# allegro/allRank

Measured on NVIDIA H100. Metric: slates/sec, higher is better.
Workload: dtype tf32

## Files before the change

allrank_b200/csrc/ffn_chain.cu:

```cuda
#include <algorithm>
#include <cstdio>
#include <cuda.h>
#include <cuda_runtime.h>

#include "common.h"
#include "gemm_tf32.h"
#include "sm90_ptx.cuh"

namespace arb {

namespace {

constexpr int CH_ROWS = 128;
constexpr int CH_UNITS = 64;
constexpr int UNIT_BYTES = 64 * 128;
constexpr int X_SLAB_BYTES = CH_ROWS * 128;
constexpr int H_SLAB_BYTES = 64 * 128;
constexpr int CH_THREADS = 384;
constexpr int SMEM_LIMIT = 227 * 1024;

template <int D>
struct ChainLayout {
  static constexpr int KB1 = D / 32;
  static constexpr int NBU = (D + 63) / 64;
  static constexpr int X_BYTES = KB1 * X_SLAB_BYTES;
  static constexpr int H_BYTES = 2 * 2 * H_SLAB_BYTES;
  static constexpr int TAIL_BYTES = 1024;
  static constexpr int NU_FIT = (SMEM_LIMIT - 1024 - TAIL_BYTES - X_BYTES - H_BYTES) / UNIT_BYTES;
  static constexpr int NU = NU_FIT < 16 ? NU_FIT : 16;
  static constexpr int RING_OFF = X_BYTES + H_BYTES;
  static constexpr int TAIL_OFF = RING_OFF + NU * UNIT_BYTES;
  static constexpr int total() { return TAIL_OFF + TAIL_BYTES + 1024; }
  static_assert(D % 32 == 0 && D >= 32 && D <= 256, "d: a multiple of 32 up to 256");
  static_assert(NU >= 2 * NBU, "the ring holds at least one k-block of the second product");
  static_assert(total() <= SMEM_LIMIT, "shared memory budget");
};

struct ChainParams {
  int M;
  int F;
  int rnd;
  int store_h;
  const float* b1;
  const float* b2;
  const float* aux;
  float* y;
  uint32_t* bits;
  float* colsum;
  const int* rows_dev;
};

__device__ __forceinline__ void load_a(uint32_t (&a)[4][4], const uint8_t* slab, int r0, int rnd) {
  const int lane = threadIdx.x & 31, j = lane >> 3;
#pragma unroll
  for (int ks = 0; ks < 4; ++ks) {
    ptx::ldmatrix_x4(a[ks], slab + ptx::sw128(r0 + 8 * (j & 1) + (lane & 7), 32 * ks + 16 * (j >> 1)));
    if (rnd) {
#pragma unroll
      for (int e = 0; e < 4; ++e) a[ks][e] = ptx::cvt_tf32(__uint_as_float(a[ks][e]));
    }
  }
}

template <int D, int U = 0>
__device__ __forceinline__ void second_mma(float (&acc)[D / 8][4], const uint32_t (&a)[4],
                                           const uint64_t (&desc)[(D + 63) / 64], int ks) {
  constexpr int WN = D % 64 == 0 ? 64 : 32;
  if constexpr (U < D / WN) {
    if constexpr (WN == 64) ptx::wgmma_m64n64k8_tf32<8 * U>(acc, a, desc[U] + 2 * ks);
    else ptx::wgmma_m64n32k8_tf32<4 * U>(acc, a, desc[U / 2] + (U & 1) * (32 * 128 / 16) + 2 * ks);
    second_mma<D, U + 1>(acc, a, desc, ks);
  }
}

template <int D, bool BWD>
__global__ void __launch_bounds__(CH_THREADS, 1) ffn_chain_kernel(const __grid_constant__ CUtensorMap tmX,
                                                                 const __grid_constant__ CUtensorMap tmA,
                                                                 const __grid_constant__ CUtensorMap tmB,
                                                                 const __grid_constant__ CUtensorMap tmH,
                                                                 const ChainParams p) {
  using L = ChainLayout<D>;
  constexpr int NU = L::NU, KB1 = L::KB1, NBU = L::NBU, NTY = D / 8;
  extern __shared__ uint8_t smem_dyn[];
  uint8_t* smem = reinterpret_cast<uint8_t*>((reinterpret_cast<uintptr_t>(smem_dyn) + 1023) & ~uintptr_t(1023));
  uint8_t* xs = smem;
  uint8_t* ring = smem + L::RING_OFF;
  uint64_t* full = reinterpret_cast<uint64_t*>(smem + L::TAIL_OFF);
  uint64_t* empty = full + NU;
  uint64_t* xfull = empty + NU;
  uint64_t* xfree = xfull + 8;
  uint64_t* csfull = xfree + 1;
  uint64_t* csempty = csfull + 2;
  float* csx = reinterpret_cast<float*>(smem + L::TAIL_OFF + 512);

  const int warp = threadIdx.x >> 5, lane = threadIdx.x & 31;
  if (threadIdx.x == 0) {
    ptx::prefetch_tmap(&tmX);
    ptx::prefetch_tmap(&tmA);
    ptx::prefetch_tmap(&tmB);
    if (p.store_h) ptx::prefetch_tmap(&tmH);
    for (int s = 0; s < NU; ++s) { ptx::mbar_init(&full[s], 1); ptx::mbar_init(&empty[s], 8); }
    for (int kb = 0; kb < KB1; ++kb) ptx::mbar_init(&xfull[kb], 1);
    ptx::mbar_init(xfree, 8);
    for (int b = 0; b < 2; ++b) { ptx::mbar_init(&csfull[b], 128); ptx::mbar_init(&csempty[b], 128); }
    ptx::fence_barrier_init();
  }
  arb_pdl_wait();
  __syncthreads();
  int n_tiles = (p.M + CH_ROWS - 1) / CH_ROWS;
  if (p.rows_dev) n_tiles = min(n_tiles, (__ldg(p.rows_dev) + CH_ROWS - 1) / CH_ROWS);
  const int n_chunks = p.F / CH_UNITS;

  if (warp >= 8) {
    asm volatile("setmaxnreg.dec.sync.aligned.u32 40;" ::: "memory");
    if (warp == 8 && lane == 0) {
      uint32_t it = 0;
      auto unit = [&](const CUtensorMap* tm, int c0, int c1) {
        const int s = it % NU;
        const uint32_t round = it / NU;
        if (round > 0) ptx::mbar_wait(&empty[s], (round - 1) & 1);
        ptx::mbar_expect_tx(&full[s], UNIT_BYTES);
        ptx::tma_load_4d(ring + s * UNIT_BYTES, tm, &full[s], c0, c1, 0, 0);
        ++it;
      };
      int local = 0;
      for (int t = blockIdx.x; t < n_tiles; t += gridDim.x, ++local) {
        const int m0 = t * CH_ROWS;
        if (local > 0) ptx::mbar_wait(xfree, (local - 1) & 1);
        for (int kb = 0; kb < KB1; ++kb) {
          ptx::mbar_expect_tx(&xfull[kb], X_SLAB_BYTES);
          ptx::tma_load_4d(xs + kb * X_SLAB_BYTES, &tmX, &xfull[kb], 32 * kb, m0, 0, 0);
        }
        if (!BWD) {
          const long long bytes = (long long)(min(p.M, m0 + CH_ROWS) - m0) * D * 4;
          asm volatile("cp.async.bulk.prefetch.L2.global [%0], %1;"
                       ::"l"(p.aux + (long long)m0 * D), "r"(uint32_t(bytes)) : "memory");
        }
        for (int j = 0; j < n_chunks; ++j) {
          for (int kb = 0; kb < KB1; ++kb) unit(&tmA, 32 * kb, CH_UNITS * j);
          for (int kb2 = 0; kb2 < 2; ++kb2)
            for (int u = 0; u < NBU; ++u) unit(&tmB, CH_UNITS * j + 32 * kb2, 64 * u);
        }
      }
    }
  } else {
    asm volatile("setmaxnreg.inc.sync.aligned.u32 232;" ::: "memory");
    const int g = warp >> 2, w = warp & 3, gq = lane >> 2, t4 = lane & 3, gt = threadIdx.x & 127;
    uint8_t* hs = smem + L::X_BYTES + g * 2 * H_SLAB_BYTES;
    const int fw = p.F >> 5;
    uint32_t it = 0, cj = 0;
    int local = 0;
    for (int t = blockIdx.x; t < n_tiles; t += gridDim.x, ++local) {
      const int m0 = t * CH_ROWS;
      const int row0 = m0 + 64 * g + 16 * w + gq;
      float accY[NTY][4];
#pragma unroll
      for (int n = 0; n < NTY; ++n) accY[n][0] = accY[n][1] = accY[n][2] = accY[n][3] = 0.f;
#pragma unroll 1
      for (int j = 0; j < n_chunks; ++j, ++cj) {
        uint32_t mw[2][2] = {{0u, 0u}, {0u, 0u}};
        if constexpr (BWD) {
#pragma unroll
          for (int h = 0; h < 2; ++h)
            if (row0 + 8 * h < p.M) {
              mw[h][0] = __ldg(p.bits + (long long)(row0 + 8 * h) * fw + 2 * j);
              mw[h][1] = __ldg(p.bits + (long long)(row0 + 8 * h) * fw + 2 * j + 1);
            }
        }
        float accH[8][4];
#pragma unroll
        for (int n = 0; n < 8; ++n) accH[n][0] = accH[n][1] = accH[n][2] = accH[n][3] = 0.f;
#pragma unroll 1
        for (int kb = 0; kb < KB1; ++kb, ++it) {
          const int s = it % NU;
          ptx::mbar_wait(&full[s], (it / NU) & 1);
          if (j == 0) ptx::mbar_wait(&xfull[kb], local & 1);
          uint32_t a[4][4];
          load_a(a, xs + kb * X_SLAB_BYTES, 64 * g + 16 * w, p.rnd);
          const uint64_t desc = ptx::wgmma_desc_sw128(ring + s * UNIT_BYTES);
          ptx::wgmma_fence_acc(accH);
          ptx::wgmma_fence();
#pragma unroll
          for (int ks = 0; ks < 4; ++ks) ptx::wgmma_m64n64k8_tf32<0>(accH, a[ks], desc + 2 * ks);
          ptx::wgmma_commit();
          ptx::wgmma_wait0();
          ptx::wgmma_fence_acc(accH);
          __syncwarp();
          if (lane == 0) ptx::mbar_arrive(&empty[s]);
        }
        if (j == n_chunks - 1) {
          __syncwarp();
          if (lane == 0) ptx::mbar_arrive(xfree);
        }
        if (p.store_h && lane == 0) ptx::tma_store_wait_read<0>();
        if (BWD && p.colsum) ptx::named_bar_sync(1 + g, 128);
        __syncwarp();
        uint32_t wb[2][2] = {{0u, 0u}, {0u, 0u}};
#pragma unroll
        for (int n = 0; n < 8; ++n) {
          const int c = 8 * n + 2 * t4, bp = 8 * (n & 3) + 2 * t4;
          float2 bb = make_float2(0.f, 0.f);
          if constexpr (!BWD) bb = __ldg(reinterpret_cast<const float2*>(p.b1 + CH_UNITS * j + c));
#pragma unroll
          for (int h = 0; h < 2; ++h) {
            float o0 = accH[n][2 * h], o1 = accH[n][2 * h + 1];
            if constexpr (BWD) {
              o0 = (mw[h][n >> 2] >> bp) & 1u ? o0 : 0.f;
              o1 = (mw[h][n >> 2] >> (bp + 1)) & 1u ? o1 : 0.f;
            } else {
              o0 += bb.x; o1 += bb.y;
              o0 = fmaxf(o0, 0.0f); o1 = fmaxf(o1, 0.0f);
              wb[h][n >> 2] |= (o0 > 0.f ? 1u : 0u) << bp | (o1 > 0.f ? 1u : 0u) << (bp + 1);
            }
            *reinterpret_cast<float2*>(hs + (n >> 2) * H_SLAB_BYTES + ptx::sw128(16 * w + gq + 8 * h, 4 * (c & 31))) =
                make_float2(o0, o1);
          }
        }
        if (!BWD && p.bits) {
#pragma unroll
          for (int h = 0; h < 2; ++h)
#pragma unroll
            for (int s = 0; s < 2; ++s) {
              wb[h][s] |= __shfl_xor_sync(0xffffffffu, wb[h][s], 1);
              wb[h][s] |= __shfl_xor_sync(0xffffffffu, wb[h][s], 2);
            }
          const int h = t4 >> 1, s = t4 & 1;
          const uint32_t word = t4 == 0 ? wb[0][0] : t4 == 1 ? wb[0][1] : t4 == 2 ? wb[1][0] : wb[1][1];
          if (row0 + 8 * h < p.M) p.bits[(long long)(row0 + 8 * h) * fw + 2 * j + s] = word;
        }
        if (p.store_h) ptx::fence_proxy_async_smem();
        __syncwarp();
        if (p.store_h && lane == 0) {
#pragma unroll
          for (int s = 0; s < 2; ++s)
            ptx::tma_store_4d(&tmH, hs + s * H_SLAB_BYTES + 16 * w * 128, CH_UNITS * j + 32 * s, m0 + 64 * g + 16 * w, 0, 0);
          ptx::tma_store_commit();
        }
        if constexpr (BWD) {
          if (p.colsum) {
            ptx::named_bar_sync(1 + g, 128);
            const int cc = gt >> 1, seg = gt & 1, c5 = cc & 31;
            const uint8_t* slab = hs + (cc >> 5) * H_SLAB_BYTES;
            float ts = 0.f;
#pragma unroll 8
            for (int r = 32 * seg; r < 32 * seg + 32; ++r)
              ts += *reinterpret_cast<const float*>(slab + r * 128 + ((((c5 >> 2) ^ (r & 7)) << 4) | ((c5 & 3) << 2)));
            ts += __shfl_xor_sync(0xffffffffu, ts, 1);
            const int b = cj & 1;
            const uint32_t use = cj >> 1;
            if (g == 1) {
              if (use > 0) ptx::mbar_wait(&csempty[b], (use - 1) & 1);
              if (seg == 0) csx[b * 64 + cc] = ts;
              ptx::mbar_arrive(&csfull[b]);
            } else {
              ptx::mbar_wait(&csfull[b], use & 1);
              const float other = csx[b * 64 + cc];
              ptx::mbar_arrive(&csempty[b]);
              if (seg == 0) p.colsum[(long long)t * p.F + CH_UNITS * j + cc] = ts + other;
            }
          }
        }
#pragma unroll 1
        for (int kb2 = 0; kb2 < 2; ++kb2, it += NBU) {
          uint32_t a[4][4];
          load_a(a, hs + kb2 * H_SLAB_BYTES, 16 * w, p.rnd);
          uint64_t desc[NBU];
#pragma unroll
          for (int u = 0; u < NBU; ++u) {
            const uint32_t iu = it + u;
            ptx::mbar_wait(&full[iu % NU], (iu / NU) & 1);
            desc[u] = ptx::wgmma_desc_sw128(ring + (iu % NU) * UNIT_BYTES);
          }
          ptx::wgmma_fence_acc(accY);
          ptx::wgmma_fence();
#pragma unroll
          for (int ks = 0; ks < 4; ++ks) second_mma<D>(accY, a[ks], desc, ks);
          ptx::wgmma_commit();
          ptx::wgmma_wait0();
          ptx::wgmma_fence_acc(accY);
          __syncwarp();
          if (lane == 0) {
#pragma unroll
            for (int u = 0; u < NBU; ++u) ptx::mbar_arrive(&empty[(it + u) % NU]);
          }
        }
      }
#pragma unroll
      for (int n0 = 0; n0 < NTY; n0 += 8) {
        constexpr int G = NTY < 8 ? NTY : 8;
        float2 r[G][2];
        if constexpr (!BWD) {
#pragma unroll
          for (int n = 0; n < G && n0 + n < NTY; ++n)
#pragma unroll
            for (int h = 0; h < 2; ++h)
              r[n][h] = row0 + 8 * h < p.M
                            ? *reinterpret_cast<const float2*>(p.aux + (long long)(row0 + 8 * h) * D + 8 * (n0 + n) + 2 * t4)
                            : make_float2(0.f, 0.f);
        }
#pragma unroll
        for (int n = 0; n < G && n0 + n < NTY; ++n) {
          const int c = 8 * (n0 + n) + 2 * t4;
          float2 bb = make_float2(0.f, 0.f);
          if constexpr (!BWD) bb = __ldg(reinterpret_cast<const float2*>(p.b2 + c));
#pragma unroll
          for (int h = 0; h < 2; ++h) {
            const int row = row0 + 8 * h;
            if (row >= p.M) continue;
            float2 o = make_float2(accY[n0 + n][2 * h], accY[n0 + n][2 * h + 1]);
            if constexpr (!BWD) {
              o.x += bb.x; o.y += bb.y;
              o.x += r[n][h].x; o.y += r[n][h].y;
            }
            *reinterpret_cast<float2*>(p.y + (long long)row * D + c) = o;
          }
        }
      }
    }
    if (p.store_h && lane == 0) ptx::tma_store_wait_all();
  }
  __syncthreads();
}

template <int D, bool BWD>
int launch_chain_t(const CUtensorMap& tX, const CUtensorMap& tA, const CUtensorMap& tB, const CUtensorMap& tH,
                   const ChainParams& p, int grid, cudaStream_t st) {
  return launch(ffn_chain_kernel<D, BWD>, dim3(grid), dim3(CH_THREADS), ChainLayout<D>::total(), st, true, tX,
                tA, tB, tH, p);
}

template <bool BWD>
int launch_chain(int d, const CUtensorMap& tX, const CUtensorMap& tA, const CUtensorMap& tB, const CUtensorMap& tH,
                 const ChainParams& p, int grid, cudaStream_t st) {
  switch (d) {
    case 32: return launch_chain_t<32, BWD>(tX, tA, tB, tH, p, grid, st);
    case 64: return launch_chain_t<64, BWD>(tX, tA, tB, tH, p, grid, st);
    case 96: return launch_chain_t<96, BWD>(tX, tA, tB, tH, p, grid, st);
    case 128: return launch_chain_t<128, BWD>(tX, tA, tB, tH, p, grid, st);
    case 160: return launch_chain_t<160, BWD>(tX, tA, tB, tH, p, grid, st);
    case 192: return launch_chain_t<192, BWD>(tX, tA, tB, tH, p, grid, st);
    case 224: return launch_chain_t<224, BWD>(tX, tA, tB, tH, p, grid, st);
    case 256: return launch_chain_t<256, BWD>(tX, tA, tB, tH, p, grid, st);
    default: arb_set_error("ffn_chain: d must be a multiple of 32 up to 256"); return ARB_E_UNSUPPORTED;
  }
}

TRef matrix(const float* p, int64_t cols, int64_t rows) {
  TRef t; t.ptr = p; t.dim[0] = cols; t.dim[1] = rows; t.stride[0] = 1; t.stride[1] = cols; return t;
}

}

bool ffn_chain_supported(int d, int f) { return d % 32 == 0 && d >= 32 && d <= 256 && f > 0 && f % CH_UNITS == 0; }

int launch_ffn_chain(const FfnChain& c, cudaStream_t st) {
  if (!ffn_chain_supported(c.d, c.f)) {
    arb_set_error("ffn_chain: needs d a multiple of 32 up to 256 and d_ff a multiple of 64");
    return ARB_E_UNSUPPORTED;
  }
  if (c.rows < 0 || !c.x || !c.a || !c.b || !c.y || (c.bwd ? !c.bits : (!c.b1 || !c.b2 || !c.aux))) {
    arb_set_error("ffn_chain: bad arguments");
    return ARB_E_INVALID_ARG;
  }
  if (c.rows == 0) return ARB_OK;
  alignas(64) CUtensorMap tX, tA, tB, tH;
  int rc;
  if ((rc = make_tmap_4d(&tX, matrix(c.x, c.d, c.rows), TmapBox{{32, CH_ROWS, 1, 1}}, 0))) return rc;
  if ((rc = make_tmap_4d(&tA, matrix(c.a, c.d, c.f), TmapBox{{32, 64, 1, 1}}, 0))) return rc;
  if ((rc = make_tmap_4d(&tB, matrix(c.b, c.f, c.d), TmapBox{{32, 64, 1, 1}}, 0))) return rc;
  if (c.h) {
    if ((rc = make_tmap_4d(&tH, matrix(c.h, c.f, c.rows), TmapBox{{32, 16, 1, 1}}, 0))) return rc;
  } else {
    tH = tX;
  }
  ChainParams p;
  p.M = c.rows; p.F = c.f; p.rnd = tf32_round_on_load(); p.store_h = c.h != nullptr;
  p.b1 = c.b1; p.b2 = c.b2; p.aux = c.aux; p.y = c.y; p.bits = c.bits; p.colsum = c.bwd ? c.colsum : nullptr;
  p.rows_dev = c.rows_dev;
  const int tiles = (c.rows + CH_ROWS - 1) / CH_ROWS;
  const int grid = std::min(tiles, sm_count());
  DetParts dp;
  dp.add(p.colsum, tiles, 1, c.f, c.f);
  if ((rc = dp.begin(st))) return rc;
  {
    const double R = double(c.rows) * (c.rows_dev ? arb_row_frac() : 1.0), d = c.d, f = c.f;
    const double bytes = 4.0 * R * d * (c.bwd ? 2.0 : 3.0) + (c.h ? 4.0 * R * f : 0.0) + (c.bits ? R * f / 8.0 : 0.0);
    char name[56];
    std::snprintf(name, sizeof name, "ffn_chain[%s M%d d%d f%d]", c.bwd ? "bwd" : "fwd", c.rows, c.d, c.f);
    ProfScope ps(ARB_PROF_GEMM, 4.0 * R * d * f, st, bytes, name);
    rc = c.bwd ? launch_chain<true>(c.d, tX, tA, tB, tH, p, grid, st) : launch_chain<false>(c.d, tX, tA, tB, tH, p, grid, st);
  }
  if (rc) return rc;
  return dp.finish(st);
}

}

extern "C" int32_t arb_ffn_forward(const float* x, const float* w1, const float* b1, const float* w2, const float* b2,
                                   const float* res, int32_t rows, int32_t d, int32_t d_ff, float* y, float* h,
                                   uint32_t* bits, const int32_t* rows_dev, void* stream) {
  arb::FfnChain c;
  c.rows = rows; c.d = d; c.f = d_ff; c.x = x; c.a = w1; c.b = w2; c.b1 = b1; c.b2 = b2; c.aux = res;
  c.y = y; c.h = h; c.bits = bits; c.rows_dev = rows_dev; c.bwd = 0;
  return arb::launch_ffn_chain(c, static_cast<cudaStream_t>(stream));
}

extern "C" int32_t arb_ffn_backward_input(const float* dy, const float* w2t, const float* w1t, const uint32_t* bits,
                                          int32_t rows, int32_t d, int32_t d_ff, float* dx, float* dh,
                                          float* grad_b1, const int32_t* rows_dev, void* stream) {
  arb::FfnChain c;
  c.rows = rows; c.d = d; c.f = d_ff; c.x = dy; c.a = w2t; c.b = w1t; c.bits = const_cast<uint32_t*>(bits);
  c.y = dx; c.h = dh; c.colsum = grad_b1; c.rows_dev = rows_dev; c.bwd = 1;
  return arb::launch_ffn_chain(c, static_cast<cudaStream_t>(stream));
}
```

allrank_b200/csrc/sm90_ptx.cuh:

```cuda
#pragma once
#include <cstdint>
#include <cuda.h>
#include <cuda_runtime.h>

namespace arb {
namespace ptx {

__device__ __forceinline__ uint32_t smem_u32(const void* p) {
  return static_cast<uint32_t>(__cvta_generic_to_shared(p));
}

__device__ __forceinline__ void mbar_init(uint64_t* bar, uint32_t count) {
  asm volatile("mbarrier.init.shared::cta.b64 [%0], %1;" ::"r"(smem_u32(bar)), "r"(count) : "memory");
}
__device__ __forceinline__ void fence_barrier_init() {
  asm volatile("fence.mbarrier_init.release.cluster;" ::: "memory");
}
__device__ __forceinline__ void mbar_expect_tx(uint64_t* bar, uint32_t bytes) {
  asm volatile("mbarrier.arrive.expect_tx.shared::cta.b64 _, [%0], %1;" ::"r"(smem_u32(bar)), "r"(bytes) : "memory");
}
__device__ __forceinline__ void mbar_arrive(uint64_t* bar) {
  asm volatile("mbarrier.arrive.shared::cta.b64 _, [%0];" ::"r"(smem_u32(bar)) : "memory");
}
__device__ __forceinline__ bool mbar_try_wait(uint64_t* bar, uint32_t parity) {
  uint32_t ok;
  asm volatile(
      "{\n\t.reg .pred p;\n\t"
      "mbarrier.try_wait.parity.shared::cta.b64 p, [%1], %2;\n\t"
      "selp.u32 %0, 1, 0, p;\n\t}"
      : "=r"(ok)
      : "r"(smem_u32(bar)), "r"(parity)
      : "memory");
  return ok != 0;
}
__device__ __forceinline__ void mbar_wait(uint64_t* bar, uint32_t parity) {
  if (mbar_try_wait(bar, parity)) return;
  const long long t0 = clock64();
  while (!mbar_try_wait(bar, parity)) {
    if (clock64() - t0 > 4000000000LL) __trap();
  }
}

__device__ __forceinline__ void fence_proxy_async_smem() {
  asm volatile("fence.proxy.async.shared::cta;" ::: "memory");
}
__device__ __forceinline__ void named_bar_sync(uint32_t id, uint32_t nthreads) {
  asm volatile("bar.sync %0, %1;" ::"r"(id), "r"(nthreads) : "memory");
}

__device__ __forceinline__ void prefetch_tmap(const CUtensorMap* m) {
  asm volatile("prefetch.tensormap [%0];" ::"l"(reinterpret_cast<uint64_t>(m)) : "memory");
}
__device__ __forceinline__ void tma_load_4d(void* dst, const CUtensorMap* m, uint64_t* bar, int c0, int c1, int c2,
                                            int c3) {
  asm volatile(
      "cp.async.bulk.tensor.4d.shared::cluster.global.mbarrier::complete_tx::bytes [%0], [%1, {%3, %4, %5, %6}], [%2];"
      ::"r"(smem_u32(dst)), "l"(reinterpret_cast<uint64_t>(m)), "r"(smem_u32(bar)), "r"(c0), "r"(c1), "r"(c2), "r"(c3)
      : "memory");
}
__device__ __forceinline__ void tma_store_4d(const CUtensorMap* m, const void* src, int c0, int c1, int c2, int c3) {
  asm volatile("cp.async.bulk.tensor.4d.global.shared::cta.bulk_group [%0, {%2, %3, %4, %5}], [%1];"
               ::"l"(reinterpret_cast<uint64_t>(m)), "r"(smem_u32(src)), "r"(c0), "r"(c1), "r"(c2), "r"(c3)
               : "memory");
}
__device__ __forceinline__ void tma_store_commit() { asm volatile("cp.async.bulk.commit_group;" ::: "memory"); }
__device__ __forceinline__ void tma_store_wait_all() { asm volatile("cp.async.bulk.wait_group 0;" ::: "memory"); }
template <int N = 0>
__device__ __forceinline__ void tma_store_wait_read() { asm volatile("cp.async.bulk.wait_group.read %0;" ::"n"(N) : "memory"); }

__device__ __forceinline__ uint32_t pack_bf16(float lo, float hi) {
  uint32_t r;
  asm("cvt.rn.bf16x2.f32 %0, %1, %2;" : "=r"(r) : "f"(hi), "f"(lo));
  return r;
}

__device__ __forceinline__ uint32_t sw128(int r, int b) {
  return uint32_t(r) * 128u + ((uint32_t((b >> 4) ^ (r & 7))) << 4) + uint32_t(b & 15);
}
__device__ __forceinline__ float4 lds128(uint32_t addr) {
  float4 v;
  asm volatile("ld.shared.v4.f32 {%0, %1, %2, %3}, [%4];" : "=f"(v.x), "=f"(v.y), "=f"(v.z), "=f"(v.w) : "r"(addr));
  return v;
}
__device__ __forceinline__ void sts128(uint32_t addr, float4 v) {
  asm volatile("st.shared.v4.f32 [%0], {%1, %2, %3, %4};" ::"r"(addr), "f"(v.x), "f"(v.y), "f"(v.z), "f"(v.w) : "memory");
}
__device__ __forceinline__ float ld_f32(const uint8_t* tile, int r, int c) {
  return *reinterpret_cast<const float*>(tile + sw128(r, 4 * c));
}

__device__ __forceinline__ uint32_t cvt_tf32(float x) {
  uint32_t r;
  asm("cvt.rn.tf32.f32 %0, %1;" : "=r"(r) : "f"(x));
  return r;
}
__device__ __forceinline__ void mma_tf32(float (&d)[4], const uint32_t (&a)[4], const uint32_t (&b)[2]) {
  asm volatile(
      "mma.sync.aligned.m16n8k8.row.col.f32.tf32.tf32.f32 {%0, %1, %2, %3}, {%4, %5, %6, %7}, {%8, %9}, "
      "{%0, %1, %2, %3};"
      : "+f"(d[0]), "+f"(d[1]), "+f"(d[2]), "+f"(d[3])
      : "r"(a[0]), "r"(a[1]), "r"(a[2]), "r"(a[3]), "r"(b[0]), "r"(b[1]));
}
__device__ __forceinline__ void mma_bf16(float (&d)[4], const uint32_t (&a)[4], const uint32_t (&b)[2]) {
  asm volatile(
      "mma.sync.aligned.m16n8k16.row.col.f32.bf16.bf16.f32 {%0, %1, %2, %3}, {%4, %5, %6, %7}, {%8, %9}, "
      "{%0, %1, %2, %3};"
      : "+f"(d[0]), "+f"(d[1]), "+f"(d[2]), "+f"(d[3])
      : "r"(a[0]), "r"(a[1]), "r"(a[2]), "r"(a[3]), "r"(b[0]), "r"(b[1]));
}
__device__ __forceinline__ void ldmatrix_x4(uint32_t (&r)[4], const void* row_addr) {
  asm volatile("ldmatrix.sync.aligned.m8n8.x4.shared.b16 {%0, %1, %2, %3}, [%4];"
               : "=r"(r[0]), "=r"(r[1]), "=r"(r[2]), "=r"(r[3])
               : "r"(smem_u32(row_addr)));
}

__device__ __forceinline__ uint64_t wgmma_desc_sw128(const void* tile) {
  const uint64_t addr = smem_u32(tile);
  return ((addr & 0x3FFFFull) >> 4) | (uint64_t(1) << 16) | (uint64_t(1024 >> 4) << 32) | (uint64_t(1) << 62);
}
__device__ __forceinline__ void wgmma_fence() { asm volatile("wgmma.fence.sync.aligned;" ::: "memory"); }
__device__ __forceinline__ void wgmma_commit() { asm volatile("wgmma.commit_group.sync.aligned;" ::: "memory"); }
__device__ __forceinline__ void wgmma_wait0() { asm volatile("wgmma.wait_group.sync.aligned 0;" ::: "memory"); }
template <int NT>
__device__ __forceinline__ void wgmma_fence_acc(float (&d)[NT][4]) {
#pragma unroll
  for (int j = 0; j < NT; ++j) asm volatile("" : "+f"(d[j][0]), "+f"(d[j][1]), "+f"(d[j][2]), "+f"(d[j][3])::"memory");
}

#define ARB_D4(j) "+f"(d[J0 + j][0]), "+f"(d[J0 + j][1]), "+f"(d[J0 + j][2]), "+f"(d[J0 + j][3])
template <int J0, int NT>
__device__ __forceinline__ void wgmma_m64n32k8_tf32(float (&d)[NT][4], const uint32_t (&a)[4], uint64_t desc_b) {
  asm volatile(
      "{\n\t.reg .pred p;\n\tsetp.ne.b32 p, %21, 0;\n\t"
      "wgmma.mma_async.sync.aligned.m64n32k8.f32.tf32.tf32 "
      "{%0, %1, %2, %3, %4, %5, %6, %7, %8, %9, %10, %11, %12, %13, %14, %15}, "
      "{%16, %17, %18, %19}, %20, p, 1, 1;\n\t}"
      : ARB_D4(0), ARB_D4(1), ARB_D4(2), ARB_D4(3)
      : "r"(a[0]), "r"(a[1]), "r"(a[2]), "r"(a[3]), "l"(desc_b), "r"(1));
}
template <int J0, int NT>
__device__ __forceinline__ void wgmma_m64n64k8_tf32(float (&d)[NT][4], const uint32_t (&a)[4], uint64_t desc_b) {
  asm volatile(
      "{\n\t.reg .pred p;\n\tsetp.ne.b32 p, %37, 0;\n\t"
      "wgmma.mma_async.sync.aligned.m64n64k8.f32.tf32.tf32 "
      "{%0, %1, %2, %3, %4, %5, %6, %7, %8, %9, %10, %11, %12, %13, %14, %15, "
      "%16, %17, %18, %19, %20, %21, %22, %23, %24, %25, %26, %27, %28, %29, %30, %31}, "
      "{%32, %33, %34, %35}, %36, p, 1, 1;\n\t}"
      : ARB_D4(0), ARB_D4(1), ARB_D4(2), ARB_D4(3), ARB_D4(4), ARB_D4(5), ARB_D4(6), ARB_D4(7)
      : "r"(a[0]), "r"(a[1]), "r"(a[2]), "r"(a[3]), "l"(desc_b), "r"(1));
}
template <int J0, int NT>
__device__ __forceinline__ void wgmma_m64n32k8_tf32_ss(float (&d)[NT][4], uint64_t desc_a, uint64_t desc_b) {
  asm volatile(
      "{\n\t.reg .pred p;\n\tsetp.ne.b32 p, %18, 0;\n\t"
      "wgmma.mma_async.sync.aligned.m64n32k8.f32.tf32.tf32 "
      "{%0, %1, %2, %3, %4, %5, %6, %7, %8, %9, %10, %11, %12, %13, %14, %15}, "
      "%16, %17, p, 1, 1;\n\t}"
      : ARB_D4(0), ARB_D4(1), ARB_D4(2), ARB_D4(3)
      : "l"(desc_a), "l"(desc_b), "r"(1));
}
template <int J0, int NT>
__device__ __forceinline__ void wgmma_m64n64k8_tf32_ss(float (&d)[NT][4], uint64_t desc_a, uint64_t desc_b) {
  asm volatile(
      "{\n\t.reg .pred p;\n\tsetp.ne.b32 p, %34, 0;\n\t"
      "wgmma.mma_async.sync.aligned.m64n64k8.f32.tf32.tf32 "
      "{%0, %1, %2, %3, %4, %5, %6, %7, %8, %9, %10, %11, %12, %13, %14, %15, "
      "%16, %17, %18, %19, %20, %21, %22, %23, %24, %25, %26, %27, %28, %29, %30, %31}, "
      "%32, %33, p, 1, 1;\n\t}"
      : ARB_D4(0), ARB_D4(1), ARB_D4(2), ARB_D4(3), ARB_D4(4), ARB_D4(5), ARB_D4(6), ARB_D4(7)
      : "l"(desc_a), "l"(desc_b), "r"(1));
}
#undef ARB_D4

__device__ __forceinline__ void acc_to_a_tf32(const float (&c)[4], uint32_t (&a)[4], int lane) {
  const int t = lane & 3, base = lane & ~3;
  const int s1 = base + (t >> 1), s2 = base + 2 + (t >> 1);
  const float x0 = __shfl_sync(0xffffffffu, c[0], s1), x1 = __shfl_sync(0xffffffffu, c[1], s1);
  const float y0 = __shfl_sync(0xffffffffu, c[2], s1), y1 = __shfl_sync(0xffffffffu, c[3], s1);
  const float u0 = __shfl_sync(0xffffffffu, c[0], s2), u1 = __shfl_sync(0xffffffffu, c[1], s2);
  const float w0 = __shfl_sync(0xffffffffu, c[2], s2), w1 = __shfl_sync(0xffffffffu, c[3], s2);
  const bool odd = (t & 1) != 0;
  a[0] = __float_as_uint(odd ? x1 : x0);
  a[1] = __float_as_uint(odd ? y1 : y0);
  a[2] = __float_as_uint(odd ? u1 : u0);
  a[3] = __float_as_uint(odd ? w1 : w0);
}

}
}
```

Measured before the change: 206,700.

## Software-pipeline FFN chain: overlap next first-product wgmma with second product

Restructures the consumer loop of the fused FFN chain into a flat step loop. The first GEMM of the next chunk is issued asynchronously, using shared-memory A operands for X, right after the second GEMM of the current chunk, so tensor-core work overlaps with the epilogue. X is rounded to TF32 once in shared memory instead of on every ldmatrix load, and accumulator zeroing is replaced by the wgmma scale-d predicate. A named-barrier turn-taking scheme between the two warpgroups is added in the backward path. This raises register pressure and synchronisation complexity, and requires the ring to hold a full chunk's units for the pipelined path.

```diff
diff --git a/allrank_b200/csrc/ffn_chain.cu b/allrank_b200/csrc/ffn_chain.cu
--- a/allrank_b200/csrc/ffn_chain.cu
+++ b/allrank_b200/csrc/ffn_chain.cu
@@ -50,6 +50,39 @@
   const int* rows_dev;
 };
 
+template <int KB1>
+__device__ __forceinline__ void round_x(uint8_t* xs, int g, int gt) {
+  const uint32_t base = ptx::smem_u32(xs) + 64 * 128 * g + 16 * gt;
+#pragma unroll
+  for (int kb = 0; kb < KB1; ++kb)
+#pragma unroll
+    for (int i = 0; i < 4; ++i) {
+      const uint32_t a = base + kb * X_SLAB_BYTES + 128 * 16 * i;
+      const float4 v = ptx::lds128(a);
+      ptx::sts128(a, make_float4(__uint_as_float(ptx::cvt_tf32(v.x)), __uint_as_float(ptx::cvt_tf32(v.y)),
+                                 __uint_as_float(ptx::cvt_tf32(v.z)), __uint_as_float(ptx::cvt_tf32(v.w))));
+    }
+  ptx::fence_proxy_async_smem();
+}
+
+template <int KB1, int NU>
+__device__ __forceinline__ void wait_units(uint64_t* full, uint32_t it) {
+#pragma unroll
+  for (int kb = 0; kb < KB1; ++kb) ptx::mbar_wait(&full[(it + kb) % NU], ((it + kb) / NU) & 1);
+}
+template <int KB1, int NU>
+__device__ __forceinline__ void first_product(float (&acc)[8][4], const uint8_t* xg, const uint8_t* ring, uint32_t it) {
+  ptx::wgmma_fence();
+#pragma unroll
+  for (int kb = 0; kb < KB1; ++kb) {
+    const uint64_t da = ptx::wgmma_desc_sw128(xg + kb * X_SLAB_BYTES);
+    const uint64_t db = ptx::wgmma_desc_sw128(ring + ((it + kb) % NU) * UNIT_BYTES);
+#pragma unroll
+    for (int ks = 0; ks < 4; ++ks) ptx::wgmma_m64n64k8_tf32_ss<0>(acc, da + 2 * ks, db + 2 * ks, kb + ks > 0);
+  }
+  ptx::wgmma_commit();
+}
+
 __device__ __forceinline__ void load_a(uint32_t (&a)[4][4], const uint8_t* slab, int r0, int rnd) {
   const int lane = threadIdx.x & 31, j = lane >> 3;
 #pragma unroll
@@ -64,12 +97,12 @@
 
 template <int D, int U = 0>
 __device__ __forceinline__ void second_mma(float (&acc)[D / 8][4], const uint32_t (&a)[4],
-                                           const uint64_t (&desc)[(D + 63) / 64], int ks) {
+                                           const uint64_t (&desc)[(D + 63) / 64], int ks, int scale_d) {
   constexpr int WN = D % 64 == 0 ? 64 : 32;
   if constexpr (U < D / WN) {
-    if constexpr (WN == 64) ptx::wgmma_m64n64k8_tf32<8 * U>(acc, a, desc[U] + 2 * ks);
-    else ptx::wgmma_m64n32k8_tf32<4 * U>(acc, a, desc[U / 2] + (U & 1) * (32 * 128 / 16) + 2 * ks);
-    second_mma<D, U + 1>(acc, a, desc, ks);
+    if constexpr (WN == 64) ptx::wgmma_m64n64k8_tf32<8 * U>(acc, a, desc[U] + 2 * ks, scale_d);
+    else ptx::wgmma_m64n32k8_tf32<4 * U>(acc, a, desc[U / 2] + (U & 1) * (32 * 128 / 16) + 2 * ks, scale_d);
+    second_mma<D, U + 1>(acc, a, desc, ks, scale_d);
   }
 }
 
@@ -145,149 +178,58 @@
     }
   } else {
     asm volatile("setmaxnreg.inc.sync.aligned.u32 232;" ::: "memory");
+    constexpr bool PIPE = KB1 + 2 * NBU <= NU;
+    constexpr int UPC = KB1 + 2 * NBU;
     const int g = warp >> 2, w = warp & 3, gq = lane >> 2, t4 = lane & 3, gt = threadIdx.x & 127;
     uint8_t* hs = smem + L::X_BYTES + g * 2 * H_SLAB_BYTES;
+    const uint8_t* xg = xs + 64 * 128 * g;
     const int fw = p.F >> 5;
-    uint32_t it = 0, cj = 0;
-    int local = 0;
-    for (int t = blockIdx.x; t < n_tiles; t += gridDim.x, ++local) {
-      const int m0 = t * CH_ROWS;
-      const int row0 = m0 + 64 * g + 16 * w + gq;
-      float accY[NTY][4];
-#pragma unroll
-      for (int n = 0; n < NTY; ++n) accY[n][0] = accY[n][1] = accY[n][2] = accY[n][3] = 0.f;
+    const int n_steps = blockIdx.x < n_tiles ? ((n_tiles - 1 - blockIdx.x) / gridDim.x + 1) * n_chunks : 0;
+    auto load_x = [&](int local) {
 #pragma unroll 1
-      for (int j = 0; j < n_chunks; ++j, ++cj) {
-        uint32_t mw[2][2] = {{0u, 0u}, {0u, 0u}};
-        if constexpr (BWD) {
-#pragma unroll
-          for (int h = 0; h < 2; ++h)
-            if (row0 + 8 * h < p.M) {
-              mw[h][0] = __ldg(p.bits + (long long)(row0 + 8 * h) * fw + 2 * j);
-              mw[h][1] = __ldg(p.bits + (long long)(row0 + 8 * h) * fw + 2 * j + 1);
-            }
-        }
-        float accH[8][4];
-#pragma unroll
-        for (int n = 0; n < 8; ++n) accH[n][0] = accH[n][1] = accH[n][2] = accH[n][3] = 0.f;
-#pragma unroll 1
-        for (int kb = 0; kb < KB1; ++kb, ++it) {
-          const int s = it % NU;
-          ptx::mbar_wait(&full[s], (it / NU) & 1);
-          if (j == 0) ptx::mbar_wait(&xfull[kb], local & 1);
-          uint32_t a[4][4];
-          load_a(a, xs + kb * X_SLAB_BYTES, 64 * g + 16 * w, p.rnd);
-          const uint64_t desc = ptx::wgmma_desc_sw128(ring + s * UNIT_BYTES);
-          ptx::wgmma_fence_acc(accH);
-          ptx::wgmma_fence();
-#pragma unroll
-          for (int ks = 0; ks < 4; ++ks) ptx::wgmma_m64n64k8_tf32<0>(accH, a[ks], desc + 2 * ks);
-          ptx::wgmma_commit();
-          ptx::wgmma_wait0();
-          ptx::wgmma_fence_acc(accH);
-          __syncwarp();
-          if (lane == 0) ptx::mbar_arrive(&empty[s]);
-        }
-        if (j == n_chunks - 1) {
-          __syncwarp();
-          if (lane == 0) ptx::mbar_arrive(xfree);
-        }
-        if (p.store_h && lane == 0) ptx::tma_store_wait_read<0>();
-        if (BWD && p.colsum) ptx::named_bar_sync(1 + g, 128);
-        __syncwarp();
-        uint32_t wb[2][2] = {{0u, 0u}, {0u, 0u}};
-#pragma unroll
-        for (int n = 0; n < 8; ++n) {
-          const int c = 8 * n + 2 * t4, bp = 8 * (n & 3) + 2 * t4;
-          float2 bb = make_float2(0.f, 0.f);
-          if constexpr (!BWD) bb = __ldg(reinterpret_cast<const float2*>(p.b1 + CH_UNITS * j + c));
-#pragma unroll
-          for (int h = 0; h < 2; ++h) {
-            float o0 = accH[n][2 * h], o1 = accH[n][2 * h + 1];
-            if constexpr (BWD) {
-              o0 = (mw[h][n >> 2] >> bp) & 1u ? o0 : 0.f;
-              o1 = (mw[h][n >> 2] >> (bp + 1)) & 1u ? o1 : 0.f;
-            } else {
-              o0 += bb.x; o1 += bb.y;
-              o0 = fmaxf(o0, 0.0f); o1 = fmaxf(o1, 0.0f);
-              wb[h][n >> 2] |= (o0 > 0.f ? 1u : 0u) << bp | (o1 > 0.f ? 1u : 0u) << (bp + 1);
-            }
-            *reinterpret_cast<float2*>(hs + (n >> 2) * H_SLAB_BYTES + ptx::sw128(16 * w + gq + 8 * h, 4 * (c & 31))) =
-                make_float2(o0, o1);
-          }
-        }
-        if (!BWD && p.bits) {
-#pragma unroll
-          for (int h = 0; h < 2; ++h)
-#pragma unroll
-            for (int s = 0; s < 2; ++s) {
-              wb[h][s] |= __shfl_xor_sync(0xffffffffu, wb[h][s], 1);
-              wb[h][s] |= __shfl_xor_sync(0xffffffffu, wb[h][s], 2);
-            }
-          const int h = t4 >> 1, s = t4 & 1;
-          const uint32_t word = t4 == 0 ? wb[0][0] : t4 == 1 ? wb[0][1] : t4 == 2 ? wb[1][0] : wb[1][1];
-          if (row0 + 8 * h < p.M) p.bits[(long long)(row0 + 8 * h) * fw + 2 * j + s] = word;
-        }
-        if (p.store_h) ptx::fence_proxy_async_smem();
-        __syncwarp();
-        if (p.store_h && lane == 0) {
-#pragma unroll
-          for (int s = 0; s < 2; ++s)
-            ptx::tma_store_4d(&tmH, hs + s * H_SLAB_BYTES + 16 * w * 128, CH_UNITS * j + 32 * s, m0 + 64 * g + 16 * w, 0, 0);
-          ptx::tma_store_commit();
-        }
-        if constexpr (BWD) {
-          if (p.colsum) {
-            ptx::named_bar_sync(1 + g, 128);
-            const int cc = gt >> 1, seg = gt & 1, c5 = cc & 31;
-            const uint8_t* slab = hs + (cc >> 5) * H_SLAB_BYTES;
-            float ts = 0.f;
-#pragma unroll 8
-            for (int r = 32 * seg; r < 32 * seg + 32; ++r)
-              ts += *reinterpret_cast<const float*>(slab + r * 128 + ((((c5 >> 2) ^ (r & 7)) << 4) | ((c5 & 3) << 2)));
-            ts += __shfl_xor_sync(0xffffffffu, ts, 1);
-            const int b = cj & 1;
-            const uint32_t use = cj >> 1;
-            if (g == 1) {
-              if (use > 0) ptx::mbar_wait(&csempty[b], (use - 1) & 1);
-              if (seg == 0) csx[b * 64 + cc] = ts;
-              ptx::mbar_arrive(&csfull[b]);
-            } else {
-              ptx::mbar_wait(&csfull[b], use & 1);
-              const float other = csx[b * 64 + cc];
-              ptx::mbar_arrive(&csempty[b]);
-              if (seg == 0) p.colsum[(long long)t * p.F + CH_UNITS * j + cc] = ts + other;
-            }
-          }
-        }
-#pragma unroll 1
-        for (int kb2 = 0; kb2 < 2; ++kb2, it += NBU) {
-          uint32_t a[4][4];
-          load_a(a, hs + kb2 * H_SLAB_BYTES, 16 * w, p.rnd);
-          uint64_t desc[NBU];
-#pragma unroll
-          for (int u = 0; u < NBU; ++u) {
-            const uint32_t iu = it + u;
-            ptx::mbar_wait(&full[iu % NU], (iu / NU) & 1);
-            desc[u] = ptx::wgmma_desc_sw128(ring + (iu % NU) * UNIT_BYTES);
-          }
-          ptx::wgmma_fence_acc(accY);
-          ptx::wgmma_fence();
-#pragma unroll
-          for (int ks = 0; ks < 4; ++ks) second_mma<D>(accY, a[ks], desc, ks);
-          ptx::wgmma_commit();
-          ptx::wgmma_wait0();
-          ptx::wgmma_fence_acc(accY);
-          __syncwarp();
-          if (lane == 0) {
-#pragma unroll
-            for (int u = 0; u < NBU; ++u) ptx::mbar_arrive(&empty[(it + u) % NU]);
-          }
-        }
-      }
-#pragma unroll
-      for (int n0 = 0; n0 < NTY; n0 += 8) {
-        constexpr int G = NTY < 8 ? NTY : 8;
+      for (int kb = 0; kb < KB1; ++kb) ptx::mbar_wait(&xfull[kb], local & 1);
+      if (p.rnd) {
+        round_x<KB1>(xs, g, gt);
+        ptx::named_bar_sync(3 + g, 128);
+      }
+    };
+    auto release = [&](uint32_t i0, int n) {
+      __syncwarp();
+      if (lane == 0)
+        for (int u = 0; u < n; ++u) ptx::mbar_arrive(&empty[(i0 + u) % NU]);
+    };
+    auto turn_begin = [&]() {
+      if constexpr (BWD) { if (g) ptx::named_bar_sync(6, 256); else ptx::named_bar_sync(5, 256); }
+    };
+    auto turn_end = [&]() {
+      if constexpr (BWD) { if (g) ptx::named_bar_arrive(5, 256); else ptx::named_bar_arrive(6, 256); }
+    };
+    if (g == 0) turn_end();
+    uint32_t mw[2][2] = {{0u, 0u}, {0u, 0u}};
+    auto load_mw = [&](int tn, int jn) {
+      const int r0 = tn * CH_ROWS + 64 * g + 16 * w + gq;
+#pragma unroll
+      for (int h = 0; h < 2; ++h) {
+        const bool in = r0 + 8 * h < p.M;
+        mw[h][0] = in ? __ldg(p.bits + (long long)(r0 + 8 * h) * fw + 2 * jn) : 0u;
+        mw[h][1] = in ? __ldg(p.bits + (long long)(r0 + 8 * h) * fw + 2 * jn + 1) : 0u;
+      }
+    };
+    float accY[NTY][4], accH[8][4];
+    int j = 0, local = 0, t = blockIdx.x;
+    if (n_steps > 0) {
+      if constexpr (BWD) load_mw(t, 0);
+      load_x(0);
+      wait_units<KB1, NU>(full, 0);
+      turn_begin();
+      first_product<KB1, NU>(accH, xg, ring, 0);
+      turn_end();
+    }
+    auto epi2 = [&]() {
+      const int row0 = t * CH_ROWS + 64 * g + 16 * w + gq;
+#pragma unroll
+      for (int n0 = 0; n0 < NTY; n0 += 4) {
+        constexpr int G = NTY < 4 ? NTY : 4;
         float2 r[G][2];
         if constexpr (!BWD) {
 #pragma unroll
@@ -316,7 +258,140 @@
           }
         }
       }
+    };
+#pragma unroll 1
+    for (int q = 0; q < n_steps; ++q) {
+      const uint32_t it = uint32_t(q) * UPC;
+      const bool last = j == n_chunks - 1, more = q + 1 < n_steps;
+      const int m0 = t * CH_ROWS;
+      const int row0 = m0 + 64 * g + 16 * w + gq;
+      ptx::wgmma_wait0();
+      ptx::wgmma_fence_acc(accH);
+      ptx::wgmma_fence_acc(accY);
+      release(it, KB1);
+      if (PIPE && j > 0) release(it - UPC + KB1, 2 * NBU);
+      if (last) {
+        __syncwarp();
+        if (lane == 0) ptx::mbar_arrive(xfree);
+      }
+      if (p.store_h && lane == 0) ptx::tma_store_wait_read<0>();
+      if (BWD && p.colsum) ptx::named_bar_sync(1 + g, 128);
+      __syncwarp();
+      uint32_t wb[2][2] = {{0u, 0u}, {0u, 0u}};
+#pragma unroll
+      for (int n = 0; n < 8; ++n) {
+        const int c = 8 * n + 2 * t4, bp = 8 * (n & 3) + 2 * t4;
+        float2 bb = make_float2(0.f, 0.f);
+        if constexpr (!BWD) bb = __ldg(reinterpret_cast<const float2*>(p.b1 + CH_UNITS * j + c));
+#pragma unroll
+        for (int h = 0; h < 2; ++h) {
+          float o0 = accH[n][2 * h], o1 = accH[n][2 * h + 1];
+          if constexpr (BWD) {
+            o0 = (mw[h][n >> 2] >> bp) & 1u ? o0 : 0.f;
+            o1 = (mw[h][n >> 2] >> (bp + 1)) & 1u ? o1 : 0.f;
+          } else {
+            o0 += bb.x; o1 += bb.y;
+            o0 = fmaxf(o0, 0.0f); o1 = fmaxf(o1, 0.0f);
+            wb[h][n >> 2] |= (o0 > 0.f ? 1u : 0u) << bp | (o1 > 0.f ? 1u : 0u) << (bp + 1);
+          }
+          *reinterpret_cast<float2*>(hs + (n >> 2) * H_SLAB_BYTES + ptx::sw128(16 * w + gq + 8 * h, 4 * (c & 31))) =
+              make_float2(o0, o1);
+        }
+      }
+      if (BWD && more) load_mw(last ? t + int(gridDim.x) : t, last ? 0 : j + 1);
+      if (!BWD && p.bits) {
+#pragma unroll
+        for (int h = 0; h < 2; ++h)
+#pragma unroll
+          for (int s = 0; s < 2; ++s) {
+            wb[h][s] |= __shfl_xor_sync(0xffffffffu, wb[h][s], 1);
+            wb[h][s] |= __shfl_xor_sync(0xffffffffu, wb[h][s], 2);
+          }
+        const int h = t4 >> 1, s = t4 & 1;
+        const uint32_t word = t4 == 0 ? wb[0][0] : t4 == 1 ? wb[0][1] : t4 == 2 ? wb[1][0] : wb[1][1];
+        if (row0 + 8 * h < p.M) p.bits[(long long)(row0 + 8 * h) * fw + 2 * j + s] = word;
+      }
+      if (p.store_h) ptx::fence_proxy_async_smem();
+      __syncwarp();
+      if (p.store_h && lane == 0) {
+#pragma unroll
+        for (int s = 0; s < 2; ++s)
+          ptx::tma_store_4d(&tmH, hs + s * H_SLAB_BYTES + 16 * w * 128, CH_UNITS * j + 32 * s, m0 + 64 * g + 16 * w, 0, 0);
+        ptx::tma_store_commit();
+      }
+      if constexpr (BWD) {
+        if (p.colsum) {
+          ptx::named_bar_sync(1 + g, 128);
+          const int cc = gt >> 1, seg = gt & 1, c5 = cc & 31;
+          const uint8_t* slab = hs + (cc >> 5) * H_SLAB_BYTES;
+          float ts = 0.f;
+#pragma unroll 8
+          for (int r = 32 * seg; r < 32 * seg + 32; ++r)
+            ts += *reinterpret_cast<const float*>(slab + r * 128 + ((((c5 >> 2) ^ (r & 7)) << 4) | ((c5 & 3) << 2)));
+          ts += __shfl_xor_sync(0xffffffffu, ts, 1);
+          const int b = q & 1;
+          const uint32_t use = uint32_t(q) >> 1;
+          if (g == 1) {
+            if (use > 0) ptx::mbar_wait(&csempty[b], (use - 1) & 1);
+            if (seg == 0) csx[b * 64 + cc] = ts;
+            ptx::mbar_arrive(&csfull[b]);
+          } else {
+            ptx::mbar_wait(&csfull[b], use & 1);
+            const float other = csx[b * 64 + cc];
+            ptx::mbar_arrive(&csempty[b]);
+            if (seg == 0) p.colsum[(long long)t * p.F + CH_UNITS * j + cc] = ts + other;
+          }
+        }
+      }
+      {
+        uint32_t a[2][4][4];
+        uint64_t desc[2][NBU];
+#pragma unroll
+        for (int kb2 = 0; kb2 < 2; ++kb2) {
+          load_a(a[kb2], hs + kb2 * H_SLAB_BYTES, 16 * w, p.rnd);
+#pragma unroll
+          for (int u = 0; u < NBU; ++u) {
+            const uint32_t iu = it + KB1 + kb2 * NBU + u;
+            ptx::mbar_wait(&full[iu % NU], (iu / NU) & 1);
+            desc[kb2][u] = ptx::wgmma_desc_sw128(ring + (iu % NU) * UNIT_BYTES);
+          }
+        }
+        if (PIPE && !last) wait_units<KB1, NU>(full, it + UPC);
+        turn_begin();
+        ptx::wgmma_fence_acc(accY);
+        ptx::wgmma_fence();
+#pragma unroll
+        for (int kb2 = 0; kb2 < 2; ++kb2)
+#pragma unroll
+          for (int ks = 0; ks < 4; ++ks) second_mma<D>(accY, a[kb2][ks], desc[kb2], ks, j > 0 || kb2 + ks > 0);
+        ptx::wgmma_commit();
+        if (PIPE && !last) first_product<KB1, NU>(accH, xg, ring, it + UPC);
+        turn_end();
+      }
+      if (!(PIPE && !last)) {
+        ptx::wgmma_wait0();
+        ptx::wgmma_fence_acc(accY);
+        release(it + KB1, 2 * NBU);
+        if (!BWD && last) epi2();
+        if (more) {
+          if (last) load_x(local + 1);
+          wait_units<KB1, NU>(full, it + UPC);
+          turn_begin();
+          first_product<KB1, NU>(accH, xg, ring, it + UPC);
+          turn_end();
+        }
+        if (BWD && last) epi2();
+      }
+      if (last) {
+        j = 0;
+        ++local;
+        t += gridDim.x;
+      } else {
+        ++j;
+      }
     }
+    ptx::wgmma_wait0();
+    if (g == 1) turn_begin();
     if (p.store_h && lane == 0) ptx::tma_store_wait_all();
   }
   __syncthreads();
diff --git a/allrank_b200/csrc/sm90_ptx.cuh b/allrank_b200/csrc/sm90_ptx.cuh
--- a/allrank_b200/csrc/sm90_ptx.cuh
+++ b/allrank_b200/csrc/sm90_ptx.cuh
@@ -46,6 +46,9 @@
 }
 __device__ __forceinline__ void named_bar_sync(uint32_t id, uint32_t nthreads) {
   asm volatile("bar.sync %0, %1;" ::"r"(id), "r"(nthreads) : "memory");
+}
+__device__ __forceinline__ void named_bar_arrive(uint32_t id, uint32_t nthreads) {
+  asm volatile("bar.arrive %0, %1;" ::"r"(id), "r"(nthreads) : "memory");
 }
 
 __device__ __forceinline__ void prefetch_tmap(const CUtensorMap* m) {
@@ -129,17 +132,19 @@
 
 #define ARB_D4(j) "+f"(d[J0 + j][0]), "+f"(d[J0 + j][1]), "+f"(d[J0 + j][2]), "+f"(d[J0 + j][3])
 template <int J0, int NT>
-__device__ __forceinline__ void wgmma_m64n32k8_tf32(float (&d)[NT][4], const uint32_t (&a)[4], uint64_t desc_b) {
+__device__ __forceinline__ void wgmma_m64n32k8_tf32(float (&d)[NT][4], const uint32_t (&a)[4], uint64_t desc_b,
+                                                    int scale_d = 1) {
   asm volatile(
       "{\n\t.reg .pred p;\n\tsetp.ne.b32 p, %21, 0;\n\t"
       "wgmma.mma_async.sync.aligned.m64n32k8.f32.tf32.tf32 "
       "{%0, %1, %2, %3, %4, %5, %6, %7, %8, %9, %10, %11, %12, %13, %14, %15}, "
       "{%16, %17, %18, %19}, %20, p, 1, 1;\n\t}"
       : ARB_D4(0), ARB_D4(1), ARB_D4(2), ARB_D4(3)
-      : "r"(a[0]), "r"(a[1]), "r"(a[2]), "r"(a[3]), "l"(desc_b), "r"(1));
+      : "r"(a[0]), "r"(a[1]), "r"(a[2]), "r"(a[3]), "l"(desc_b), "r"(scale_d));
 }
 template <int J0, int NT>
-__device__ __forceinline__ void wgmma_m64n64k8_tf32(float (&d)[NT][4], const uint32_t (&a)[4], uint64_t desc_b) {
+__device__ __forceinline__ void wgmma_m64n64k8_tf32(float (&d)[NT][4], const uint32_t (&a)[4], uint64_t desc_b,
+                                                    int scale_d = 1) {
   asm volatile(
       "{\n\t.reg .pred p;\n\tsetp.ne.b32 p, %37, 0;\n\t"
       "wgmma.mma_async.sync.aligned.m64n64k8.f32.tf32.tf32 "
@@ -147,20 +152,22 @@
       "%16, %17, %18, %19, %20, %21, %22, %23, %24, %25, %26, %27, %28, %29, %30, %31}, "
       "{%32, %33, %34, %35}, %36, p, 1, 1;\n\t}"
       : ARB_D4(0), ARB_D4(1), ARB_D4(2), ARB_D4(3), ARB_D4(4), ARB_D4(5), ARB_D4(6), ARB_D4(7)
-      : "r"(a[0]), "r"(a[1]), "r"(a[2]), "r"(a[3]), "l"(desc_b), "r"(1));
+      : "r"(a[0]), "r"(a[1]), "r"(a[2]), "r"(a[3]), "l"(desc_b), "r"(scale_d));
 }
 template <int J0, int NT>
-__device__ __forceinline__ void wgmma_m64n32k8_tf32_ss(float (&d)[NT][4], uint64_t desc_a, uint64_t desc_b) {
+__device__ __forceinline__ void wgmma_m64n32k8_tf32_ss(float (&d)[NT][4], uint64_t desc_a, uint64_t desc_b,
+                                                    int scale_d = 1) {
   asm volatile(
       "{\n\t.reg .pred p;\n\tsetp.ne.b32 p, %18, 0;\n\t"
       "wgmma.mma_async.sync.aligned.m64n32k8.f32.tf32.tf32 "
       "{%0, %1, %2, %3, %4, %5, %6, %7, %8, %9, %10, %11, %12, %13, %14, %15}, "
       "%16, %17, p, 1, 1;\n\t}"
       : ARB_D4(0), ARB_D4(1), ARB_D4(2), ARB_D4(3)
-      : "l"(desc_a), "l"(desc_b), "r"(1));
+      : "l"(desc_a), "l"(desc_b), "r"(scale_d));
 }
 template <int J0, int NT>
-__device__ __forceinline__ void wgmma_m64n64k8_tf32_ss(float (&d)[NT][4], uint64_t desc_a, uint64_t desc_b) {
+__device__ __forceinline__ void wgmma_m64n64k8_tf32_ss(float (&d)[NT][4], uint64_t desc_a, uint64_t desc_b,
+                                                    int scale_d = 1) {
   asm volatile(
       "{\n\t.reg .pred p;\n\tsetp.ne.b32 p, %34, 0;\n\t"
       "wgmma.mma_async.sync.aligned.m64n64k8.f32.tf32.tf32 "
@@ -168,7 +175,7 @@
       "%16, %17, %18, %19, %20, %21, %22, %23, %24, %25, %26, %27, %28, %29, %30, %31}, "
       "%32, %33, p, 1, 1;\n\t}"
       : ARB_D4(0), ARB_D4(1), ARB_D4(2), ARB_D4(3), ARB_D4(4), ARB_D4(5), ARB_D4(6), ARB_D4(7)
-      : "l"(desc_a), "l"(desc_b), "r"(1));
+      : "l"(desc_a), "l"(desc_b), "r"(scale_d));
 }
 #undef ARB_D4
 
```

Measured after the change: 209,700, median of 6. 1.4% higher.
